# kleinzcy/speech_signal_processing

Hardware: NVIDIA B200
Metric: frames/sec MFCC+GMM-UBM scoring (1024 comp) (higher is better)
Workload: dtype f16 operands (11-bit significand, as tf32) / f32 accumulate; common part 3-pass f32 grade

## Files before the change

### speech_signal_processing_b200/csrc/gmm_score_sv.cu

```cuda
#include <cuda_fp16.h>

#include <cstdlib>

#include "tc_common.cuh"

namespace ssp {
namespace sv {
using namespace tc;

constexpr int BM = 128;
constexpr int MB = 2;
constexpr int UNIT = BM * MB;
static_assert(UNIT == kSvUnit, "sv_smem_bytes");
constexpr int BN = kSvTileN;
constexpr int NSTAGE = kSvStages;
constexpr int NSLOT = kSvSlots;
constexpr int EPI_WARPS = 16;
constexpr int EPI = EPI_WARPS * 32;
constexpr int CTRL = 128;
constexpr int THREADS = CTRL + EPI;
constexpr int CTRL_REGS = 32, EPI_REGS = 112;
constexpr int NQ = kSvBaseImages;
constexpr int CHUNK = kSvChunk;
constexpr uint32_t ACC_COL0 = 128;
constexpr uint32_t kRelaxNs = 1000;
constexpr int kPolyPairs = 6;
constexpr int kPolyDeg = 3;

struct Args {
  const float* feats;
  const int64_t* offsets;
  int64_t n_utts, total_frames;
  const __half* tiles;
  const __half* tiles_group;
  int n_models;
  int set_images;
  int set_models;
  int n_tiles, D, KS, normalize;
  int KQ;
  float* stab;
  double* scores;
  float* frame_lse;
};

__device__ __forceinline__ void named_bar_sync(int id, int n) { asm volatile("bar.sync %0, %1;" ::"r"(id), "r"(n) : "memory"); }

__device__ __forceinline__ bool bar_try_wait(uint32_t bar, uint32_t parity) {
  uint32_t ok;
  asm volatile(
      "{\n\t.reg .pred p;\n\t"
      "mbarrier.try_wait.parity.shared::cta.b64 p, [%1], %2;\n\t"
      "selp.u32 %0, 1, 0, p;\n\t}"
      : "=r"(ok)
      : "r"(bar), "r"(parity)
      : "memory");
  return ok != 0;
}
__device__ __forceinline__ void bar_spin(uint32_t bar, uint32_t parity) {
  if (bar_try_wait(bar, parity)) return;
  const long long t0 = clock64();
  while (!bar_try_wait(bar, parity)) {
    if (clock64() - t0 > (1ll << 31)) __trap();
  }
}
__device__ __forceinline__ void bar_spin_relaxed(uint32_t bar, uint32_t parity) {
  if (bar_try_wait(bar, parity)) return;
  const long long t0 = clock64();
  for (;;) {
    uint32_t ok;
    asm volatile(
        "{\n\t.reg .pred p;\n\t"
        "mbarrier.try_wait.parity.shared::cta.b64 p, [%1], %2, %3;\n\t"
        "selp.u32 %0, 1, 0, p;\n\t}"
        : "=r"(ok)
        : "r"(bar), "r"(parity), "r"(kRelaxNs)
        : "memory");
    if (ok) return;
    if (clock64() - t0 > (1ll << 31)) __trap();
  }
}
__device__ __forceinline__ void bar_arrive(uint32_t bar) {
  asm volatile("mbarrier.arrive.shared::cta.b64 _, [%0];" ::"r"(bar) : "memory");
}
__device__ __forceinline__ void bar_arrive_expect_tx(uint32_t bar, uint32_t bytes) {
  asm volatile("mbarrier.arrive.expect_tx.shared::cta.b64 _, [%0], %1;" ::"r"(bar), "r"(bytes) : "memory");
}
__device__ __forceinline__ void bar_commit(uint32_t bar) {
  asm volatile("tcgen05.commit.cta_group::1.mbarrier::arrive::one.shared::cluster.b64 [%0];" ::"r"(bar) : "memory");
}
__device__ __forceinline__ void bulk_g2s_u32(uint32_t smem_dst, const void* gmem_src, uint32_t bytes, uint32_t bar) {
  asm volatile("cp.async.bulk.shared::cluster.global.mbarrier::complete_tx::bytes [%0], [%1], %2, [%3];" ::"r"(smem_dst),
               "l"(gmem_src), "r"(bytes), "r"(bar)
               : "memory");
}

__device__ __forceinline__ void tc_st8(uint32_t taddr, const uint32_t (&r)[8]) {
  asm volatile("tcgen05.st.sync.aligned.32x32b.x8.b32 [%0], {%1, %2, %3, %4, %5, %6, %7, %8};" ::"r"(taddr), "r"(r[0]),
               "r"(r[1]), "r"(r[2]), "r"(r[3]), "r"(r[4]), "r"(r[5]), "r"(r[6]), "r"(r[7])
               : "memory");
}

__device__ __forceinline__ float exp_sum32(const uint32_t (&r)[32], const float (&qm)[32]) {
  static_assert(kPolyPairs % 2 == 0 && kPolyPairs <= 16, "pairs are consumed two at a time");
  static_assert(kPolyDeg == 3, "the coefficients below are those of the degree-3 polynomial");
  const float MAGIC = 12582912.f;
  const float2 mg = make_float2(MAGIC, MAGIC), nmg = make_float2(-MAGIC, -MAGIC), neg1 = make_float2(-1.f, -1.f);
  float2 accp = make_float2(0.f, 0.f), accm0 = accp, accm1 = accp;
#pragma unroll
  for (int i = 0; i < kPolyPairs; ++i) {
    float2 d = make_float2(__uint_as_float(r[2 * i]), __uint_as_float(r[2 * i + 1]));
    d.x = fmaxf(d.x, -126.f);
    d.y = fmaxf(d.y, -126.f);
    const float2 t = __fadd2_rn(d, mg);
    const float2 nn = __fadd2_rn(t, nmg);
    const float2 f = __ffma2_rn(nn, neg1, d);
    float2 p = __ffma2_rn(make_float2(0.0551716685295105f, 0.0551716685295105f), f, make_float2(0.2426111251115799f, 0.2426111251115799f));
    p = __ffma2_rn(p, f, make_float2(0.6932609677314758f, 0.6932609677314758f));
    p = __ffma2_rn(p, f, make_float2(0.9999280571937561f, 0.9999280571937561f));
    float2 e;
    e.x = __uint_as_float(__float_as_uint(p.x) + (__float_as_uint(t.x) << 23));
    e.y = __uint_as_float(__float_as_uint(p.y) + (__float_as_uint(t.y) << 23));
    accp = __ffma2_rn(e, make_float2(qm[2 * i], qm[2 * i + 1]), accp);
  }
#pragma unroll
  for (int i = kPolyPairs; i < 16; i += 2) {
    const float2 d0 = make_float2(__uint_as_float(r[2 * i]), __uint_as_float(r[2 * i + 1]));
    const float2 d1 = make_float2(__uint_as_float(r[2 * i + 2]), __uint_as_float(r[2 * i + 3]));
    accm0 = __ffma2_rn(make_float2(ex2(d0.x), ex2(d0.y)), make_float2(qm[2 * i], qm[2 * i + 1]), accm0);
    accm1 = __ffma2_rn(make_float2(ex2(d1.x), ex2(d1.y)), make_float2(qm[2 * i + 2], qm[2 * i + 3]), accm1);
  }
  const float2 tot = __fadd2_rn(__fadd2_rn(accm0, accm1), accp);
  return tot.x + tot.y;
}

template <int KSTEPS, bool kFirst>
__global__ void __launch_bounds__(THREADS, 1) gmm_score_sv_kernel(const Args a) {
  extern __shared__ __align__(1024) unsigned char smem[];
  constexpr int KS = KSTEPS * 16;
  constexpr uint32_t tile_bytes = (uint32_t)BN * KS * 2u;
  const uint32_t aq_block_bytes = (uint32_t)a.KQ * BM * 2u;
  __half* sAh = reinterpret_cast<__half*>(smem);
  __half* sAl = reinterpret_cast<__half*>(smem + (size_t)MB * aq_block_bytes);
  unsigned char* sB = smem + (size_t)2 * MB * aq_block_bytes;
  float* sPart = reinterpret_cast<float*>(sB + (size_t)NSTAGE * tile_bytes);
  uint64_t* bars = reinterpret_cast<uint64_t*>(sPart + 2 * CHUNK * UNIT);
  const uint32_t b_full = smem_u32(bars);
  const uint32_t b_empty = b_full + 8u * NSTAGE;
  const uint32_t t_full = b_empty + 8u * NSTAGE;
  const uint32_t t_empty = t_full + 8u * NSLOT;
  const uint32_t a_full = t_empty + 8u * NSLOT;
  const uint32_t a_empty = a_full + 8u;
  uint32_t* tmem_slot = reinterpret_cast<uint32_t*>(bars + 2 * NSTAGE + 2 * NSLOT + 2);
  float* mstab = reinterpret_cast<float*>(tmem_slot + 4);
  float* mx = sPart;

  const int tid = threadIdx.x, warp = tid >> 5, lane = tid & 31;

  if (tid == 0) {
    for (int i = 0; i < NSTAGE; ++i) { mbar_init(bars + i, 1); mbar_init(bars + NSTAGE + i, MB); }
    for (int i = 0; i < NSLOT; ++i) { mbar_init(bars + 2 * NSTAGE + i, 1); mbar_init(bars + 2 * NSTAGE + NSLOT + i, EPI_WARPS / MB); }
    mbar_init(bars + 2 * NSTAGE + 2 * NSLOT, EPI);
    mbar_init(bars + 2 * NSTAGE + 2 * NSLOT + 1, MB);
    asm volatile("fence.mbarrier_init.release.cluster;" ::: "memory");
  }
  if (warp == 1) {
    asm volatile("tcgen05.alloc.cta_group::1.sync.aligned.shared::cta.b32 [%0], %1;" ::"r"(smem_u32(tmem_slot)), "r"(512u)
                 : "memory");
    asm volatile("tcgen05.relinquish_alloc_permit.cta_group::1.sync.aligned;" ::: "memory");
  }
  if (tid >= CTRL)
    for (int i = tid - CTRL; i < 2 * CHUNK * UNIT; i += EPI) sPart[i] = 0.f;
  tc_fence_before();
  __syncthreads();
  tc_fence_after();
  const uint32_t tmem_base = *tmem_slot;

  const int64_t n_units = (a.total_frames + UNIT - 1) / UNIT;
  const int S = a.n_models, NT = a.n_tiles;
  constexpr size_t tile_halfs = (size_t)BN * KS;

  if (warp < CTRL / 32) {
    asm volatile("setmaxnreg.dec.sync.aligned.u32 %0;" ::"n"(CTRL_REGS));
  if (warp == 0) {
    const uint32_t sB_u32 = smem_u32(sB);
    uint32_t stage = 0, ph = 0;
    auto load = [&](const __half* src) {
      bar_spin_relaxed(b_empty + 8u * stage, ph ^ 1u);
      if (elect_one()) {
        bar_arrive_expect_tx(b_full + 8u * stage, tile_bytes);
        bulk_g2s_u32(sB_u32 + stage * tile_bytes, src, tile_bytes, b_full + 8u * stage);
      }
      __syncwarp();
      if (++stage == NSTAGE) { stage = 0; ph ^= 1u; }
    };
    const size_t tile_stride = (size_t)a.set_images * tile_halfs;
    for (int64_t u = blockIdx.x; u < n_units; u += gridDim.x) {
      if (kFirst)
        for (int j = 0; j < NT; ++j) {
          const __half* tj = a.tiles + (size_t)j * tile_stride;
          for (int i = 0; i < NQ; ++i, tj += tile_halfs) load(tj);
        }
      for (int m0 = 0; m0 < S; m0 += CHUNK) {
        const int nm = min(CHUNK, S - m0);
        for (int j = 0; j < NT; ++j) {
          const __half* tj = a.tiles + (size_t)j * tile_stride;
          for (int i = 0; i < NQ; ++i, tj += tile_halfs) load(tj);
          const __half* src = a.tiles_group + (size_t)j * tile_stride + (size_t)(NQ + m0) * tile_halfs;
          for (int m = 0; m < nm; ++m, src += tile_halfs) load(src);
        }
      }
    }
  } else if (warp == 1 || warp == 2) {
    const int g = warp - 1;
    constexpr uint32_t lbo_a = BM * 16u, lbo_b = BN * 16u, sbo = 128u;
    constexpr uint32_t ks_a = (2u * lbo_a) >> 4, ks_b = (2u * lbo_b) >> 4;
    constexpr uint32_t tile_units = tile_bytes >> 4;
    const uint64_t ah_desc = make_desc(smem_u32(sAh) + (uint32_t)g * aq_block_bytes, lbo_a, sbo);
    const uint64_t al_desc = make_desc(smem_u32(sAl) + (uint32_t)g * aq_block_bytes, lbo_a, sbo);
    const uint64_t b_desc0 = make_desc(smem_u32(sB), lbo_b, sbo);
    const uint32_t at = tmem_base + (uint32_t)(g * (KS / 2));
    constexpr uint32_t idesc = make_idesc_f16(BM, BN);
    const int steps_b = (a.KQ - KS) >> 4;
    uint32_t stage = 0, bph = 0, s3 = 0, sph = 0, unit_idx = 0;
    auto next_stage = [&]() { if (++stage == NSTAGE) { stage = 0; bph ^= 1u; } };
    auto next_slot = [&]() { if (++s3 == 3) { s3 = 0; sph ^= 1u; } };
    auto job_r = [&]() {
      bar_spin_relaxed(b_full + 8u * stage, bph);
      const uint32_t slot = (uint32_t)g + 2u * s3;
      bar_spin_relaxed(t_empty + 8u * slot, sph ^ 1u);
      tc_fence_after();
      if (elect_one()) {
        const uint32_t d_tmem = tmem_base + ACC_COL0 + slot * BN;
        const uint64_t bd = b_desc0 + (uint64_t)(stage * tile_units);
#pragma unroll
        for (int k = 0; k < KSTEPS; ++k) mma_f16_ts(d_tmem, at + 8u * k, bd + (uint64_t)(k * ks_b), idesc, k > 0 ? 1u : 0u);
        bar_commit(t_full + 8u * slot);
        bar_commit(b_empty + 8u * stage);
      }
      __syncwarp();
      next_stage();
      next_slot();
    };
    auto job_q = [&]() {
      const uint32_t slot = (uint32_t)g + 2u * s3;
      bar_spin_relaxed(t_empty + 8u * slot, sph ^ 1u);
      const uint32_t d_tmem = tmem_base + ACC_COL0 + slot * BN;
#pragma unroll
      for (int part = 0; part < NQ; ++part) {
        bar_spin_relaxed(b_full + 8u * stage, bph);
        tc_fence_after();
        if (elect_one()) {
          const uint64_t bd = b_desc0 + (uint64_t)(stage * tile_units);
          const bool second = (part & 1) != 0;
          const uint64_t a_off = second ? (uint64_t)(KSTEPS * ks_a) : 0ull;
#pragma unroll
          for (int k = 0; k < KSTEPS; ++k)
            if (!second || k < steps_b)
              mma_f16_ss(d_tmem, ah_desc + a_off + (uint64_t)(k * ks_a), bd + (uint64_t)(k * ks_b), idesc, (part | k) ? 1u : 0u);
          if (part < 2) {
#pragma unroll
            for (int k = 0; k < KSTEPS; ++k)
              if (!second || k < steps_b)
                mma_f16_ss(d_tmem, al_desc + a_off + (uint64_t)(k * ks_a), bd + (uint64_t)(k * ks_b), idesc, 1u);
          }
          if (part == NQ - 1) bar_commit(t_full + 8u * slot);
          bar_commit(b_empty + 8u * stage);
        }
        __syncwarp();
        next_stage();
      }
      next_slot();
    };
    for (int64_t u = blockIdx.x; u < n_units; u += gridDim.x, ++unit_idx) {
      bar_spin_relaxed(a_full, unit_idx & 1u);
      tc_fence_after();
      if (kFirst)
        for (int j = 0; j < NT; ++j) job_q();
      for (int m0 = 0; m0 < S; m0 += CHUNK) {
        const int nm = min(CHUNK, S - m0);
        for (int j = 0; j < NT; ++j) {
          job_q();
#pragma unroll 1
          for (int m = 0; m < nm; ++m) job_r();
        }
      }
      if (elect_one()) bar_commit(a_empty);
      __syncwarp();
    }
  }
  } else {
    asm volatile("setmaxnreg.inc.sync.aligned.u32 %0;" ::"n"(EPI_REGS));
    const int etid = tid - CTRL;
    const int ew = warp - CTRL / 32;
    const int quad = warp & 3;
    const int g = (ew >> 2) & 1;
    const int half = ew >> 3;
    const int row = quad * 32 + lane;
    const int urow = g * BM + row;
    const uint32_t lane_addr = (uint32_t)(quad * 32) << 16;
    const int frow = etid & (UNIT - 1), fpart = etid >> 8;
    const float LN2 = 0.69314718055994530942f;
    float* my_part = sPart + (size_t)half * CHUNK * UNIT + urow;
    uint32_t s3 = 0, sph = 0, unit_idx = 0;

    const uint32_t my_tmem = tmem_base + lane_addr + ACC_COL0 + (uint32_t)(g * BN + half * 32);
    const uint32_t my_full = t_full + 8u * g, my_empty = t_empty + 8u * g;
    const bool lane0 = lane == 0;
    auto fetch = [&](uint32_t (&r)[32]) {
      bar_spin(my_full + 16u * s3, sph);
      tc_fence_after();
      tc_ld32_issue(my_tmem + 2u * BN * s3, r);
      tc_ld_wait(r);
      tc_fence_before();
      __syncwarp();
      if (lane0) bar_arrive(my_empty + 16u * s3);
      if (++s3 == 3) { s3 = 0; sph ^= 1u; }
    };

    for (int64_t u = blockIdx.x; u < n_units; u += gridDim.x, ++unit_idx) {
      const int64_t frame0 = u * UNIT;
      bar_spin(a_empty, (unit_idx & 1u) ^ 1u);
      tc_fence_after();
      {
        const int64_t fr = frame0 + frow;
        const bool live = fr < a.total_frames;
        const float* xr = a.feats + fr * a.D;
        const size_t at0 = (size_t)(frow >> 7) * (BM * a.KQ) + (size_t)(frow & (BM - 1)) * 8;
        const int j0 = fpart * (a.KQ >> 1), j1 = j0 + (a.KQ >> 1);
        for (int j = j0; j < j1; ++j) {
          float y = 0.f;
          if (j < 2 * a.D) {
            if (live) { const float x = xr[j < a.D ? j : j - a.D]; y = j < a.D ? x * x : x; }
          } else if (j < 2 * a.D + 2) {
            y = 1.f;
          }
          const __half h = __float2half_rn(y);
          const size_t at1 = at0 + (size_t)(j >> 3) * (BM * 8) + (j & 7);
          sAh[at1] = h;
          sAl[at1] = __float2half_rn(y - __half2float(h));
        }
      }
      {
        const int64_t fe = frame0 + urow;
        const bool live = fe < a.total_frames;
        const float* xr = a.feats + fe * a.D;
        for (int c = half; c < KSTEPS; c += 2) {
          uint32_t v[8];
#pragma unroll
          for (int e = 0; e < 8; ++e) {
            float x2[2];
#pragma unroll
            for (int i = 0; i < 2; ++i) {
              const int j = 16 * c + 2 * e + i;
              float x = 0.f;
              if (j < a.D) x = live ? xr[j] : 0.f;
              else if (j == a.D) x = 1.f;
              else if (j == a.D + 1) x = kSvConstScale;
              x2[i] = x;
            }
            const __half2 hh = __floats2half2_rn(x2[0], x2[1]);
            v[e] = *reinterpret_cast<const uint32_t*>(&hh);
          }
          tc_st8(tmem_base + lane_addr + (uint32_t)(g * (KS / 2) + 8 * c), v);
        }
        asm volatile("tcgen05.wait::st.sync.aligned;" ::: "memory");
      }
      asm volatile("fence.proxy.async.shared::cta;" ::: "memory");
      tc_fence_before();
      bar_arrive(a_full);

      const int64_t ff = frame0 + frow;
      const bool flive = ff < a.total_frames;
      const int futt = flive ? find_segment(a.offsets, a.n_utts, ff) : -1;
      float fwgt = 1.f;
      if (futt >= 0 && a.normalize) fwgt = 1.f / (float)(a.offsets[futt + 1] - a.offsets[futt]);

      float m_t;
      if (kFirst) {
        float rmax = -3.0e38f;
        for (int j = 0; j < NT; ++j) {
          uint32_t r[32];
          fetch(r);
          float cm = max3(__uint_as_float(r[0]), __uint_as_float(r[1]), __uint_as_float(r[2]));
#pragma unroll
          for (int i = 3; i < 31; i += 2) cm = max3(cm, __uint_as_float(r[i]), __uint_as_float(r[i + 1]));
          rmax = max3(rmax, cm, __uint_as_float(r[31]));
        }
        mx[half * UNIT + urow] = rmax;
        named_bar_sync(1 + g, 2 * BM);
        m_t = rintf(fmaxf(mx[urow], mx[UNIT + urow]));
        named_bar_sync(1 + g, 2 * BM);
        if (half == 0) { mx[urow] = 0.f; mx[UNIT + urow] = 0.f; }
        if (half == 0 && a.stab && frame0 + urow < a.total_frames) a.stab[frame0 + urow] = m_t;
      } else {
        m_t = frame0 + urow < a.total_frames ? a.stab[frame0 + urow] : 0.f;
      }
      if (half == 0) mstab[urow] = m_t;

      for (int m0 = 0; m0 < S; m0 += CHUNK) {
        const int nm = min(CHUNK, S - m0);
        for (int j = 0; j < NT; ++j) {
          float qm[32];
          {
            uint32_t r[32];
            fetch(r);
#pragma unroll
            for (int i = 0; i < 32; ++i) qm[i] = ex2(__uint_as_float(r[i]) - m_t);
          }
          float* dst = my_part;
#pragma unroll 1
          for (int m = 0; m < nm; ++m, dst += UNIT) {
            uint32_t r[32];
            fetch(r);
            *dst += exp_sum32(r, qm);
          }
        }
        named_bar_sync(3, EPI);
        {
          const float mf = mstab[frow];
          float* p0 = sPart + (size_t)fpart * UNIT + frow;
          for (int m = fpart; m < nm; m += 2, p0 += 2 * UNIT) {
            const float v = p0[0] + p0[CHUNK * UNIT];
            p0[0] = 0.f;
            p0[CHUNK * UNIT] = 0.f;
            float lse = (mf + lg2(v)) * LN2;
            if (!(v > 7.9e-31f && v < 1.2e30f)) lse = __int_as_float(0x7fc00000);
            if (flive && a.frame_lse) a.frame_lse[(int64_t)(m0 + m) * a.total_frames + ff] = lse;
            warp_segmented_atomic_add(a.scores, futt, a.set_models, m0 + m, lse * fwgt, lane);
          }
        }
        named_bar_sync(3, EPI);
      }
    }
  }

  tc_fence_before();
  __syncthreads();
  if (warp == 1) asm volatile("tcgen05.dealloc.cta_group::1.sync.aligned.b32 %0, %1;" ::"r"(tmem_base), "r"(512u) : "memory");
}

__global__ void __launch_bounds__(256) sv_fixup_kernel(const Args a, int64_t n_pairs) {
  const int lane = threadIdx.x & 31;
  const int64_t warp0 = ((int64_t)blockIdx.x * blockDim.x + threadIdx.x) >> 5;
  const int64_t n_warps = ((int64_t)gridDim.x * blockDim.x) >> 5;
  const int S = a.set_models, KS = a.KS, KQ = a.KQ, D = a.D;
  const size_t tile_halfs = (size_t)BN * KS;
  const float LN2 = 0.69314718055994530942f;
  for (int64_t p = warp0; p < n_pairs; p += n_warps) {
    const double cur = a.scores[p];
    if (cur == cur && fabs(cur) < 1.0e300) continue;
    const int64_t utt = p / S;
    const int m = (int)(p % S);
    const int64_t t0 = a.offsets[utt], t1 = a.offsets[utt + 1];
    double total = 0.0;
    for (int64_t t = t0; t < t1; ++t) {
      const float* xr = a.feats + t * D;
      float mrun = -3.0e38f, srun = 0.f;
      for (int c = lane; c < a.n_tiles * BN; c += 32) {
        const __half* tq = a.tiles + ((size_t)(c / BN) * (S + NQ)) * tile_halfs;
        const __half* tr = tq + (size_t)(NQ + m) * tile_halfs;
        const int n = c % BN;
        auto at = [&](const __half* tile, int j) { return __half2float(tile[((size_t)(j >> 3) * BN + n) * 8 + (j & 7)]); };
        auto bq = [&](int j) {
          const __half* t_hi = j < KS ? tq : tq + tile_halfs;
          const int jj = j < KS ? j : j - KS;
          return at(t_hi, jj) + at(t_hi + 2 * tile_halfs, jj);
        };
        float l = at(tr, D) + kSvConstScale * at(tr, D + 1);
        for (int j = 2 * D; j < KQ; ++j) l += bq(j);
        for (int j = 0; j < D; ++j) {
          const float x = xr[j];
          l = fmaf(x, at(tr, j) + bq(D + j), l);
          l = fmaf(x * x, bq(j), l);
        }
        const float mn = fmaxf(mrun, l);
        srun = srun * exp2f(mrun - mn) + exp2f(l - mn);
        mrun = mn;
      }
      const float mall = warp_max(mrun);
      const float sall = warp_sum(srun * exp2f(mrun - mall));
      const float lse = (mall + log2f(sall)) * LN2;
      if (lane == 0 && a.frame_lse) a.frame_lse[(int64_t)m * a.total_frames + t] = lse;
      total += (double)lse;
    }
    if (lane == 0) a.scores[p] = a.normalize && t1 > t0 ? total / (double)(t1 - t0) : total;
  }
}

static int g_num_sms = 0;
static int num_sms() {
  if (g_num_sms == 0) {
    int dev = 0;
    if (cudaGetDevice(&dev) != cudaSuccess || cudaDeviceGetAttribute(&g_num_sms, cudaDevAttrMultiProcessorCount, dev) != cudaSuccess)
      g_num_sms = 148;
  }
  return g_num_sms;
}

template <int KSTEPS>
static int launch_one(const Args& a, unsigned grid, bool first, cudaStream_t st) {
  const size_t smem = sv_smem_bytes(KSTEPS * 16, a.KQ);
  if (first) {
    SSP_CUDA_OK(cudaFuncSetAttribute(gmm_score_sv_kernel<KSTEPS, true>, cudaFuncAttributeMaxDynamicSharedMemorySize, (int)smem));
    gmm_score_sv_kernel<KSTEPS, true><<<grid, THREADS, smem, st>>>(a);
  } else {
    SSP_CUDA_OK(cudaFuncSetAttribute(gmm_score_sv_kernel<KSTEPS, false>, cudaFuncAttributeMaxDynamicSharedMemorySize, (int)smem));
    gmm_score_sv_kernel<KSTEPS, false><<<grid, THREADS, smem, st>>>(a);
  }
  return SSP_OK;
}
static int launch_ks(const Args& a, unsigned grid, bool first, cudaStream_t st) {
  switch (a.KS) {
    case 16: return launch_one<1>(a, grid, first, st);
    case 32: return launch_one<2>(a, grid, first, st);
    case 48: return launch_one<3>(a, grid, first, st);
    case 64: return launch_one<4>(a, grid, first, st);
  }
  set_error("ssp_gmm_score_shared: contraction length %d is not a multiple of 16 in [16, 64]", a.KS);
  return SSP_EINVAL;
}

}

static int sv_group_models(const SvLayout& L) {
  static double mb = -1.0;
  if (mb < 0.0) {
    const char* e = getenv("SSP_SV_GROUP_MB");
    mb = e ? atof(e) : 48.0;
  }
  if (mb <= 0.0) return L.n_models;
  const double per_model = (double)L.Kp * L.KS * 2.0;
  int cap = (int)(mb * 1048576.0 / per_model) / sv::CHUNK * sv::CHUNK;
  if (cap < sv::CHUNK) cap = sv::CHUNK;
  if (cap >= L.n_models) return L.n_models;
  const int n_groups = (L.n_models + cap - 1) / cap;
  int g = ((L.n_models + n_groups - 1) / n_groups + sv::CHUNK - 1) / sv::CHUNK * sv::CHUNK;
  return g >= L.n_models ? L.n_models : g;
}

int64_t score_sv_workspace_bytes(const SvLayout& L, int64_t total_frames) {
  return sv_group_models(L) < L.n_models ? (int64_t)sizeof(float) * total_frames : 0;
}

int launch_score_sv(const float* feats, const int64_t* offsets, int64_t n_utts, int64_t total_frames, const void* pack,
                    const SvLayout& L, bool normalize, double* scores, float* frame_lse, void* workspace, cudaStream_t st) {
  using namespace sv;
  SSP_CUDA_OK(cudaMemsetAsync(scores, 0, sizeof(double) * n_utts * L.n_models, st));
  if (total_frames == 0) return SSP_OK;
  const int group = sv_group_models(L);
  Args a;
  a.feats = feats;
  a.offsets = offsets;
  a.n_utts = n_utts;
  a.total_frames = total_frames;
  a.tiles = (const __half*)pack;
  a.set_images = L.n_models + NQ;
  a.set_models = L.n_models;
  a.n_tiles = L.Kp / BN;
  a.D = L.D;
  a.KS = L.KS;
  a.KQ = L.KQ;
  a.normalize = normalize ? 1 : 0;
  a.stab = group < L.n_models ? (float*)workspace : nullptr;
  const int64_t n_units = (total_frames + UNIT - 1) / UNIT;
  const unsigned grid = (unsigned)(n_units < num_sms() ? n_units : num_sms());
  for (int m0 = 0; m0 < L.n_models; m0 += group) {
    a.n_models = L.n_models - m0 < group ? L.n_models - m0 : group;
    a.tiles_group = a.tiles + (size_t)m0 * BN * L.KS;
    a.scores = scores + m0;
    a.frame_lse = frame_lse ? frame_lse + (size_t)m0 * total_frames : nullptr;
    const int rc = launch_ks(a, grid, m0 == 0, st);
    if (rc != SSP_OK) return rc;
    SSP_LAUNCH_CHECK("gmm_score_sv_kernel");
  }
  a.n_models = L.n_models;
  a.tiles_group = a.tiles;
  a.scores = scores;
  a.frame_lse = frame_lse;
  const int64_t n_pairs = n_utts * L.n_models;
  const int64_t want = (n_pairs + 7) / 8, cap = 4 * (int64_t)num_sms();
  sv_fixup_kernel<<<(unsigned)(want < cap ? want : cap), 256, 0, st>>>(a, n_pairs);
  SSP_LAUNCH_CHECK("sv_fixup_kernel");
  return SSP_OK;
}

}
```

Baseline: 4.429 million.

## Pair model-score accumulators in TMEM to halve barrier handshakes per model

TMEM accumulator slots change from three rotating single-tile slots per group to one dedicated query slot plus a two-tile pair slot. The MMA warp now issues two model tiles into the pair before one commit, and the epilogue loads both with two in-flight TMEM loads and a single barrier release. This is meant to cut mbarrier round-trips and to overlap the two TMEM loads. The cost is less buffering depth: there is a single pair slot, not three rotating slots, which may expose MMA/epilogue stalls. The per-frame utterance lookup is also moved into the chunk reduction, so it is recomputed per chunk, which trims register pressure in the main loop.

Result: faster. 4.710 million (median of 6 runs) (+6.4%).

```diff
diff --git a/speech_signal_processing_b200/csrc/gmm_score_sv.cu b/speech_signal_processing_b200/csrc/gmm_score_sv.cu
--- a/speech_signal_processing_b200/csrc/gmm_score_sv.cu
+++ b/speech_signal_processing_b200/csrc/gmm_score_sv.cu
@@ -15,6 +15,8 @@
 constexpr int BN = kSvTileN;
 constexpr int NSTAGE = kSvStages;
 constexpr int NSLOT = kSvSlots;
+static_assert(NSLOT == 3 * MB, "slot layout");
+constexpr int NACC = 2 * MB;
 constexpr int EPI_WARPS = 16;
 constexpr int EPI = EPI_WARPS * 32;
 constexpr int CTRL = 128;
@@ -23,6 +25,8 @@
 constexpr int NQ = kSvBaseImages;
 constexpr int CHUNK = kSvChunk;
 constexpr uint32_t ACC_COL0 = 128;
+constexpr uint32_t PAIR_COL0 = ACC_COL0 + MB * BN;
+static_assert(PAIR_COL0 + MB * 2 * BN == 512 && ACC_COL0 + NSLOT * BN == 512, "TMEM columns");
 constexpr uint32_t kRelaxNs = 1000;
 constexpr int kPolyPairs = 6;
 constexpr int kPolyDeg = 3;
@@ -147,10 +151,10 @@
   const uint32_t b_full = smem_u32(bars);
   const uint32_t b_empty = b_full + 8u * NSTAGE;
   const uint32_t t_full = b_empty + 8u * NSTAGE;
-  const uint32_t t_empty = t_full + 8u * NSLOT;
-  const uint32_t a_full = t_empty + 8u * NSLOT;
+  const uint32_t t_empty = t_full + 8u * NACC;
+  const uint32_t a_full = t_empty + 8u * NACC;
   const uint32_t a_empty = a_full + 8u;
-  uint32_t* tmem_slot = reinterpret_cast<uint32_t*>(bars + 2 * NSTAGE + 2 * NSLOT + 2);
+  uint32_t* tmem_slot = reinterpret_cast<uint32_t*>(bars + 2 * NSTAGE + 2 * NACC + 2);
   float* mstab = reinterpret_cast<float*>(tmem_slot + 4);
   float* mx = sPart;
 
@@ -158,9 +162,9 @@
 
   if (tid == 0) {
     for (int i = 0; i < NSTAGE; ++i) { mbar_init(bars + i, 1); mbar_init(bars + NSTAGE + i, MB); }
-    for (int i = 0; i < NSLOT; ++i) { mbar_init(bars + 2 * NSTAGE + i, 1); mbar_init(bars + 2 * NSTAGE + NSLOT + i, EPI_WARPS / MB); }
-    mbar_init(bars + 2 * NSTAGE + 2 * NSLOT, EPI);
-    mbar_init(bars + 2 * NSTAGE + 2 * NSLOT + 1, MB);
+    for (int i = 0; i < NACC; ++i) { mbar_init(bars + 2 * NSTAGE + i, 1); mbar_init(bars + 2 * NSTAGE + NACC + i, EPI_WARPS / MB); }
+    mbar_init(bars + 2 * NSTAGE + 2 * NACC, EPI);
+    mbar_init(bars + 2 * NSTAGE + 2 * NACC + 1, MB);
     asm volatile("fence.mbarrier_init.release.cluster;" ::: "memory");
   }
   if (warp == 1) {
@@ -221,30 +225,34 @@
     const uint32_t at = tmem_base + (uint32_t)(g * (KS / 2));
     constexpr uint32_t idesc = make_idesc_f16(BM, BN);
     const int steps_b = (a.KQ - KS) >> 4;
-    uint32_t stage = 0, bph = 0, s3 = 0, sph = 0, unit_idx = 0;
+    uint32_t stage = 0, bph = 0, qph = 0, pph = 0, unit_idx = 0;
     auto next_stage = [&]() { if (++stage == NSTAGE) { stage = 0; bph ^= 1u; } };
-    auto next_slot = [&]() { if (++s3 == 3) { s3 = 0; sph ^= 1u; } };
-    auto job_r = [&]() {
-      bar_spin_relaxed(b_full + 8u * stage, bph);
-      const uint32_t slot = (uint32_t)g + 2u * s3;
-      bar_spin_relaxed(t_empty + 8u * slot, sph ^ 1u);
-      tc_fence_after();
-      if (elect_one()) {
-        const uint32_t d_tmem = tmem_base + ACC_COL0 + slot * BN;
-        const uint64_t bd = b_desc0 + (uint64_t)(stage * tile_units);
-#pragma unroll
-        for (int k = 0; k < KSTEPS; ++k) mma_f16_ts(d_tmem, at + 8u * k, bd + (uint64_t)(k * ks_b), idesc, k > 0 ? 1u : 0u);
-        bar_commit(t_full + 8u * slot);
-        bar_commit(b_empty + 8u * stage);
-      }
-      __syncwarp();
-      next_stage();
-      next_slot();
+    const uint32_t q_full = t_full + 8u * g, q_empty = t_empty + 8u * g;
+    const uint32_t p_full = t_full + 8u * (MB + g), p_empty = t_empty + 8u * (MB + g);
+    const uint32_t p_tmem = tmem_base + PAIR_COL0 + (uint32_t)g * 2u * BN;
+    auto job_r = [&](const bool two) {
+      bar_spin_relaxed(p_empty, pph ^ 1u);
+#pragma unroll
+      for (int i = 0; i < 2; ++i) {
+        if (i == 1 && !two) break;
+        bar_spin_relaxed(b_full + 8u * stage, bph);
+        tc_fence_after();
+        if (elect_one()) {
+          const uint32_t d_tmem = p_tmem + (uint32_t)i * BN;
+          const uint64_t bd = b_desc0 + (uint64_t)(stage * tile_units);
+#pragma unroll
+          for (int k = 0; k < KSTEPS; ++k) mma_f16_ts(d_tmem, at + 8u * k, bd + (uint64_t)(k * ks_b), idesc, k > 0 ? 1u : 0u);
+          if (i == 1 || !two) bar_commit(p_full);
+          bar_commit(b_empty + 8u * stage);
+        }
+        __syncwarp();
+        next_stage();
+      }
+      pph ^= 1u;
     };
     auto job_q = [&]() {
-      const uint32_t slot = (uint32_t)g + 2u * s3;
-      bar_spin_relaxed(t_empty + 8u * slot, sph ^ 1u);
-      const uint32_t d_tmem = tmem_base + ACC_COL0 + slot * BN;
+      bar_spin_relaxed(q_empty, qph ^ 1u);
+      const uint32_t d_tmem = tmem_base + ACC_COL0 + (uint32_t)g * BN;
 #pragma unroll
       for (int part = 0; part < NQ; ++part) {
         bar_spin_relaxed(b_full + 8u * stage, bph);
@@ -263,13 +271,13 @@
               if (!second || k < steps_b)
                 mma_f16_ss(d_tmem, al_desc + a_off + (uint64_t)(k * ks_a), bd + (uint64_t)(k * ks_b), idesc, 1u);
           }
-          if (part == NQ - 1) bar_commit(t_full + 8u * slot);
+          if (part == NQ - 1) bar_commit(q_full);
           bar_commit(b_empty + 8u * stage);
         }
         __syncwarp();
         next_stage();
       }
-      next_slot();
+      qph ^= 1u;
     };
     for (int64_t u = blockIdx.x; u < n_units; u += gridDim.x, ++unit_idx) {
       bar_spin_relaxed(a_full, unit_idx & 1u);
@@ -281,7 +289,7 @@
         for (int j = 0; j < NT; ++j) {
           job_q();
 #pragma unroll 1
-          for (int m = 0; m < nm; ++m) job_r();
+          for (int m = 0; m < nm; m += 2) job_r(m + 1 < nm);
         }
       }
       if (elect_one()) bar_commit(a_empty);
@@ -301,20 +309,26 @@
     const int frow = etid & (UNIT - 1), fpart = etid >> 8;
     const float LN2 = 0.69314718055994530942f;
     float* my_part = sPart + (size_t)half * CHUNK * UNIT + urow;
-    uint32_t s3 = 0, sph = 0, unit_idx = 0;
-
-    const uint32_t my_tmem = tmem_base + lane_addr + ACC_COL0 + (uint32_t)(g * BN + half * 32);
-    const uint32_t my_full = t_full + 8u * g, my_empty = t_empty + 8u * g;
+    uint32_t qph = 0, pph = 0, unit_idx = 0;
+
+    const uint32_t q_tmem = tmem_base + lane_addr + ACC_COL0 + (uint32_t)(g * BN + half * 32);
+    const uint32_t p_col = lane_addr + PAIR_COL0 + (uint32_t)(g * 2 * BN + half * 32);
+    const volatile uint32_t* tmem_base_smem = tmem_slot;
+    const uint32_t q_full = t_full + 8u * g, q_empty = t_empty + 8u * g;
+    const uint32_t p_full = t_full + 8u * (MB + g), p_empty = t_empty + 8u * (MB + g);
     const bool lane0 = lane == 0;
-    auto fetch = [&](uint32_t (&r)[32]) {
-      bar_spin(my_full + 16u * s3, sph);
-      tc_fence_after();
-      tc_ld32_issue(my_tmem + 2u * BN * s3, r);
-      tc_ld_wait(r);
+    auto release = [&](uint32_t empty) {
       tc_fence_before();
       __syncwarp();
-      if (lane0) bar_arrive(my_empty + 16u * s3);
-      if (++s3 == 3) { s3 = 0; sph ^= 1u; }
+      if (lane0) bar_arrive(empty);
+    };
+    auto fetch_q = [&](uint32_t (&r)[32]) {
+      bar_spin(q_full, qph);
+      tc_fence_after();
+      tc_ld32_issue(q_tmem, r);
+      tc_ld_wait(r);
+      release(q_empty);
+      qph ^= 1u;
     };
 
     for (int64_t u = blockIdx.x; u < n_units; u += gridDim.x, ++unit_idx) {
@@ -369,18 +383,12 @@
       tc_fence_before();
       bar_arrive(a_full);
 
-      const int64_t ff = frame0 + frow;
-      const bool flive = ff < a.total_frames;
-      const int futt = flive ? find_segment(a.offsets, a.n_utts, ff) : -1;
-      float fwgt = 1.f;
-      if (futt >= 0 && a.normalize) fwgt = 1.f / (float)(a.offsets[futt + 1] - a.offsets[futt]);
-
       float m_t;
       if (kFirst) {
         float rmax = -3.0e38f;
         for (int j = 0; j < NT; ++j) {
           uint32_t r[32];
-          fetch(r);
+          fetch_q(r);
           float cm = max3(__uint_as_float(r[0]), __uint_as_float(r[1]), __uint_as_float(r[2]));
 #pragma unroll
           for (int i = 3; i < 31; i += 2) cm = max3(cm, __uint_as_float(r[i]), __uint_as_float(r[i + 1]));
@@ -403,20 +411,43 @@
           float qm[32];
           {
             uint32_t r[32];
-            fetch(r);
+            fetch_q(r);
 #pragma unroll
             for (int i = 0; i < 32; ++i) qm[i] = ex2(__uint_as_float(r[i]) - m_t);
           }
           float* dst = my_part;
 #pragma unroll 1
-          for (int m = 0; m < nm; ++m, dst += UNIT) {
+          for (int m = 1; m < nm; m += 2, dst += 2 * UNIT) {
+            uint32_t r0[32], r1[32];
+            const uint32_t p_tmem = *tmem_base_smem + p_col;
+            bar_spin(p_full, pph);
+            tc_fence_after();
+            tc_ld32_issue(p_tmem, r0);
+            tc_ld32_issue(p_tmem + BN, r1);
+            tc_ld_wait2(r0, r1);
+            release(p_empty);
+            pph ^= 1u;
+            dst[0] += exp_sum32(r0, qm);
+            dst[UNIT] += exp_sum32(r1, qm);
+          }
+          if (nm & 1) {
             uint32_t r[32];
-            fetch(r);
+            bar_spin(p_full, pph);
+            tc_fence_after();
+            tc_ld32_issue(*tmem_base_smem + p_col, r);
+            tc_ld_wait(r);
+            release(p_empty);
+            pph ^= 1u;
             *dst += exp_sum32(r, qm);
           }
         }
         named_bar_sync(3, EPI);
         {
+          const int64_t ff = frame0 + frow;
+          const bool flive = ff < a.total_frames;
+          const int futt = flive ? find_segment(a.offsets, a.n_utts, ff) : -1;
+          float fwgt = 1.f;
+          if (futt >= 0 && a.normalize) fwgt = 1.f / (float)(a.offsets[futt + 1] - a.offsets[futt]);
           const float mf = mstab[frow];
           float* p0 = sPart + (size_t)fpart * UNIT + frow;
           for (int m = fpart; m < nm; m += 2, p0 += 2 * UNIT) {
```
